# humanlongevity/tredparse

Measured on AMD Instinct MI355X. Metric: sample x TRED genotypes/sec at 30x 150bp, higher is better.
Workload: dtype int32 (SW) + f64 (likelihood)

## Files before the change

tredparse_amd/csrc/capi.hip:

```cpp
#include <algorithm>
#include <cstdarg>
#include <cstdio>
#include <cmath>
#include <cstdlib>
#include <cstring>
#include <ctime>
#include <string>
#include <vector>

#include <unistd.h>

#include "tredgpu_internal.h"
#include "inflater_internal.h"
#include "kmer_host.h"

using namespace tredgpu;

namespace {

struct Buf {
    void* p = nullptr;
    size_t cap = 0;
};

std::string g_create_error;

}

struct tredgpu_ctx {
    int device = 0;
    hipStream_t stream = nullptr;
    std::string err;
    std::vector<LadderDesc> h_ladders;
    Buf d_ladders, d_seq;
    int max_ladder_units = 0;
    Buf d_model;
    bool have_model = false;
    Buf ws_quads, ws_counter, ws_drop, ws_stats, ws_perm, ws_class, ws_ucnt, ws_bins, ws_best, ws_cnt;
    struct GridBufs { Buf pool, descs, items, counters, kde, unit_max; } grid;
    int* h_pin = nullptr;
    hipEvent_t sync_ev = nullptr;
    size_t grid_pool_bytes = GRID_POOL_BYTES;
    std::vector<Buf> st;
    struct PinBlock { uint8_t* p; size_t cap, used; };
    std::vector<PinBlock> pin;
    struct PinOut { void* host; const void* pinned; size_t bytes; };
    std::vector<PinOut> pin_out;
    struct Timer {
        std::vector<std::pair<hipEvent_t, hipEvent_t>> pool;
        size_t used = 0;
        int64_t launches = 0;
        double total_ms = 0;
    } timers[7];
};

namespace {

int fail(tredgpu_ctx* c, int code, const char* fmt, ...) {
    char buf[512];
    va_list ap;
    va_start(ap, fmt);
    vsnprintf(buf, sizeof buf, fmt, ap);
    va_end(ap);
    if (c) c->err = buf; else g_create_error = buf;
    return code;
}

int hip_rc(tredgpu_ctx* c, hipError_t e, const char* what) {
    return e == hipSuccess ? 0 : fail(c, -10, "%s: %s", what, hipGetErrorString(e));
}

#define HIPRC(c, expr) hip_rc((c), (expr), #expr)
#define HIPCHK(c, expr)                          \
    do {                                         \
        if (int rc_ = HIPRC(c, expr)) return rc_; \
    } while (0)

void timer_flush(tredgpu_ctx::Timer& t) {
    for (size_t i = 0; i < t.used; ++i) {
        float ms = 0;
        if (hipEventElapsedTime(&ms, t.pool[i].first, t.pool[i].second) == hipSuccess) {
            t.total_ms += ms;
            t.launches += 1;
        }
    }
    t.used = 0;
}

struct ScopedTimer {
    tredgpu_ctx* c;
    tredgpu_ctx::Timer& t;
    hipEvent_t stop = nullptr;
    ScopedTimer(tredgpu_ctx* c_, int which) : c(c_), t(c_->timers[which]) {
        if (t.used >= 256) {
            (void)hipStreamSynchronize(c->stream);
            timer_flush(t);
        }
        if (t.used == t.pool.size()) {
            hipEvent_t a = nullptr, b = nullptr;
            if (hipEventCreate(&a) != hipSuccess || hipEventCreate(&b) != hipSuccess) return;
            t.pool.emplace_back(a, b);
        }
        (void)hipEventRecord(t.pool[t.used].first, c->stream);
        stop = t.pool[t.used].second;
    }
    ~ScopedTimer() {
        if (stop) {
            (void)hipEventRecord(stop, c->stream);
            t.used += 1;
        }
    }
};

void* pin_alloc(tredgpu_ctx* c, size_t bytes) {
    bytes = (bytes + 63) & ~(size_t)63;
    for (auto& b : c->pin)
        if (b.cap - b.used >= bytes) { void* at = b.p + b.used; b.used += bytes; return at; }
    size_t cap = std::max<size_t>(bytes, (size_t)8 << 20);
    if (!c->pin.empty()) cap = std::max(cap, c->pin.back().cap * 2);
    uint8_t* p = nullptr;
    if (hipHostMalloc((void**)&p, cap, hipHostMallocDefault) != hipSuccess) return nullptr;
// ... 143 lines not shown
        const Staged& a = list[k];
        if (!a.dst || !a.bytes) continue;
        void* h;
        if ((rc = pin_for(c, a.bytes, &h))) break;
        rc = HIPRC(c, hipMemcpyAsync(h, c->st[k].p, a.bytes, hipMemcpyDeviceToHost, c->stream));
        if (!rc) c->pin_out.push_back({a.dst, h, a.bytes});
    }
    if (rc) {
        (void)stream_sync(c, false);
        return rc;
    }
    return HIPRC(c, stream_sync(c));
}

int check_unit(tredgpu_ctx* c, int g, const tredgpu_unit_params& u, const int32_t* unit_ladder, int32_t hist_stride,
               int64_t n_global_total, int64_t n_target_total, int32_t marg_stride, int limits[2]) {
    if (unit_ladder) {
        const int lad = unit_ladder[g];
        if (lad < 0 || lad >= (int)c->h_ladders.size()) return fail(c, -2, "unit %d: ladder %d not registered", g, lad);
        if (hist_stride <= c->h_ladders[lad].max_units)
            return fail(c, -2, "hist_stride %d must exceed the max_units %d of unit %d's ladder", hist_stride, c->h_ladders[lad].max_units, g);
    }
    limits[0] = std::max(limits[0], u.maxinsert);
    limits[1] = std::max(limits[1], u.n_target);
    if (u.n_global < 0 || u.n_target < 0 || u.pe_off < 0 || u.tl_off < 0 || (int64_t)u.pe_off + u.n_global > n_global_total ||
        (int64_t)u.tl_off + u.n_target > n_target_total)
        return fail(c, -2, "unit %d: paired-end slices out of range", g);
    if (marg_stride > 0 && marg_stride <= std::max(u.maxinsert, hist_stride)) return fail(c, -2, "marg_stride must exceed max(maxinsert, hist_stride)");
    return 0;
}

int host_max_len(tredgpu_ctx* c, const tredgpu_sw_params* p, const int32_t* read_len, int64_t n_reads, int* max_len) {
    int seen = 0;
    for (int64_t r = 0; r < n_reads; ++r) seen = std::max(seen, read_len[r]);
    if (seen > TREDGPU_MAX_READ_LEN) return fail(c, -5, "read of %d bp exceeds TREDGPU_MAX_READ_LEN=%d", seen, TREDGPU_MAX_READ_LEN);
    *max_len = std::max(p->max_read_len > 0 ? p->max_read_len : seen, 1);
    return check_sw_range(c, p, *max_len);
}

}

extern "C" {

#ifndef TREDGPU_SRC_HASH
#define TREDGPU_SRC_HASH "unknown"
#endif
const char* tredgpu_version(void) { return "tredgpu 0.6 (gfx950) src " TREDGPU_SRC_HASH; }

int tredgpu_create(int device_id, tredgpu_ctx** out) {
    if (!out) return fail(nullptr, -2, "out is NULL");
    *out = nullptr;
    int n = 0;
    hipError_t e = hipGetDeviceCount(&n);
    if (e != hipSuccess || n <= 0)
        return fail(nullptr, -3, "no HIP device available (%s); libtredgpu has no CPU fallback",
                    e == hipSuccess ? "device count 0" : hipGetErrorString(e));
    if (device_id < 0 || device_id >= n) return fail(nullptr, -2, "device %d out of range [0,%d)", device_id, n);
    tredgpu_ctx* c = new tredgpu_ctx();
    c->device = device_id;
    int lo_prio = 0, hi_prio = 0;
    const char* want = getenv("TREDGPU_CTX_PRIORITY");
    const bool high = want && strcmp(want, "high") == 0;
    const char* split = getenv("TREDGPU_CTX_CUS");
    if ((e = hipSetDevice(device_id)) != hipSuccess ||
        (e = (split && atoi(split) > 0) ? tredgpu_front::create_partitioned_stream(&c->stream, hipStreamDefault, 0, 1, device_id)
             : high && hipDeviceGetStreamPriorityRange(&lo_prio, &hi_prio) == hipSuccess
                 ? hipStreamCreateWithPriority(&c->stream, hipStreamDefault, hi_prio) : hipStreamCreate(&c->stream)) != hipSuccess) {
        delete c;
        return fail(nullptr, -10, "cannot initialise device %d: %s", device_id, hipGetErrorString(e));
    }
    if (const char* mb = getenv("TREDGPU_GRID_POOL_MB")) {
        const long v = atol(mb);
        if (v > 0) c->grid_pool_bytes = (size_t)v << 20;
    }
    *out = c;
    return 0;
}

void tredgpu_destroy(tredgpu_ctx* c) {
    if (!c) return;
    (void)hipSetDevice(c->device);
    (void)stream_sync(c);
    for (Buf* b : {&c->d_ladders, &c->d_seq, &c->d_model, &c->ws_quads, &c->ws_counter, &c->ws_drop,
                   &c->ws_stats, &c->ws_perm, &c->ws_class, &c->ws_ucnt, &c->ws_bins, &c->ws_best, &c->ws_cnt, &c->grid.pool, &c->grid.descs,
                   &c->grid.items, &c->grid.counters, &c->grid.kde, &c->grid.unit_max})
        release(*b);
    for (Buf& b : c->st) release(b);
    for (auto& t : c->timers)
        for (auto& ev : t.pool) { (void)hipEventDestroy(ev.first); (void)hipEventDestroy(ev.second); }
    if (c->h_pin) (void)hipHostFree(c->h_pin);
    if (c->sync_ev) (void)hipEventDestroy(c->sync_ev);
    for (auto& b : c->pin) (void)hipHostFree(b.p);
    c->pin.clear();
    (void)hipStreamDestroy(c->stream);
    delete c;
}

const char* tredgpu_last_error(const tredgpu_ctx* c) { return c ? c->err.c_str() : g_create_error.c_str(); }

int tredgpu_sync(tredgpu_ctx* c) {
    if (!c) return -2;
    HIPCHK(c, hipSetDevice(c->device));
    HIPCHK(c, stream_sync(c));
    return 0;
}

void* tredgpu_get_stream(tredgpu_ctx* c) { return c ? (void*)c->stream : nullptr; }

int tredgpu_reset_timing(tredgpu_ctx* c) {
    if (!c) return -2;
    HIPCHK(c, hipSetDevice(c->device));
    HIPCHK(c, stream_sync(c));
    for (auto& t : c->timers) { t.used = 0; t.launches = 0; t.total_ms = 0; }
    if (c->ws_stats.p) HIPCHK(c, hipMemsetAsync(c->ws_stats.p, 0, SW_STAT_SLOTS * 8 * sizeof(unsigned long long), c->stream));
    return 0;
}

int tredgpu_get_sw_counters(tredgpu_ctx* c, uint64_t out[8]) {
    if (!c || !out) return -2;
    HIPCHK(c, hipSetDevice(c->device));
    for (int i = 0; i < 8; ++i) out[i] = 0;
    if (c->ws_stats.p) {
        std::vector<uint64_t> slots((size_t)SW_STAT_SLOTS * 8);
        HIPCHK(c, hipMemcpyAsync(slots.data(), c->ws_stats.p, slots.size() * sizeof(uint64_t), hipMemcpyDeviceToHost, c->stream));
        HIPCHK(c, stream_sync(c));
        for (int k = 0; k < SW_STAT_SLOTS; ++k)
            for (int i = 0; i < 8; ++i) out[i] += slots[(size_t)k * 8 + i];
    }
    HIPCHK(c, stream_sync(c));
    return 0;
}

int tredgpu_get_timing(tredgpu_ctx* c, int which, int64_t* launches, double* total_ms) {
    if (!c) return -2;
    if (which < 0 || which > 6) return fail(c, -2, "which must be one of TREDGPU_KERNEL_*");
    HIPCHK(c, hipSetDevice(c->device));
    HIPCHK(c, stream_sync(c));
    timer_flush(c->timers[which]);
    if (launches) *launches = c->timers[which].launches;
    if (total_ms) *total_ms = c->timers[which].total_ms;
    return 0;
}

int tredgpu_set_ladders(tredgpu_ctx* c, int32_t n, const char* const* prefix, const char* const* repeat,
                        const char* const* suffix, const int32_t* max_units) {
    if (!c) return -2;
    if (n < 0 || (n > 0 && (!prefix || !repeat || !suffix || !max_units))) return fail(c, -2, "bad ladder arguments");
    HIPCHK(c, hipSetDevice(c->device));
    std::vector<uint32_t> seq;
    auto append = [&seq](const std::vector<int8_t>& v) {
        const int off = (int)seq.size();
        seq.resize(seq.size() + (v.size() + 7) / 8 + 1, 0x44444444u);
        for (size_t i = 0; i < v.size(); ++i) {
            uint32_t& w = seq[off + i / 8];
            w = (w & ~(0xFu << ((i % 8) * 4))) | ((uint32_t)v[i] << ((i % 8) * 4));
        }
        return off;
    };
    std::vector<LadderDesc> lad((size_t)n);
    int max_u = 0;
    for (int i = 0; i < n; ++i) {
        std::vector<int8_t> P, Rp, S;
        encode(prefix[i], P);
        encode(repeat[i], Rp);
        encode(suffix[i], S);
        const int mu = max_units[i];
        LadderDesc& d = lad[i];
// ... 61 lines not shown
    HIPCHK(c, hipSetDevice(c->device));
    std::vector<ModelConst> mbuf(1);
    ModelConst& m = mbuf[0];
    memcpy(m.step, step_pdf, sizeof m.step);
    memcpy(m.w, stutter_w, sizeof m.w);
    m.gc = gc;
    m.score = score;
    m.small = std::exp(-10.0);
    m.really_small = std::exp(-100.0);
    m.logsmall = std::log(m.small);
    for (int n = 0; n < GRID_LFACT; ++n) m.lfact[n] = std::lgamma((double)n + 1);
    int rc;
    if ((rc = ensure(c, c->d_model, sizeof m))) return rc;
    HIPCHK(c, stream_sync(c));
    HIPCHK(c, hipMemcpy(c->d_model.p, &m, sizeof m, hipMemcpyHostToDevice));
    c->have_model = true;
    return 0;
}

int64_t tredgpu_pack_reads(const char* seqs, const int64_t* seq_off, int64_t n_reads, uint32_t* packed_out,
                           int64_t* word_off_out, int32_t* len_out) {
    if (n_reads < 0 || (n_reads > 0 && (!seqs || !seq_off))) return -2;
    int64_t w = 0;
    for (int64_t r = 0; r < n_reads; ++r) {
        const int64_t L = seq_off[r + 1] - seq_off[r];
        if (L < 0 || L > 0x7fffffff) return -2;
        const int64_t nb = (L + 15) >> 4, nm = (L + 31) >> 5;
        if (word_off_out) word_off_out[r] = w;
        if (len_out) len_out[r] = (int32_t)L;
        if (packed_out) {
            uint32_t* rec = packed_out + w;
            for (int64_t k = 0; k < nb + nm; ++k) rec[k] = 0;
            const char* s = seqs + seq_off[r];
            for (int64_t i = 0; i < L; ++i) {
                const int code = base_code(s[i]);
                if (code == 4) rec[nb + (i >> 5)] |= 1u << (i & 31);
                else rec[i >> 4] |= (uint32_t)code << ((i & 15) * 2);
            }
        }
        w += nb + nm;
    }
    if (word_off_out) word_off_out[n_reads] = w;
    return w;
}


static int run_sw_device(tredgpu_ctx* c, const uint32_t* packed, const int64_t* read_off, const int32_t* read_len,
                         int64_t n_reads, const int32_t* unit_read_off, const int32_t* unit_ladder,
                         int32_t n_units, const tredgpu_sw_params* p, int max_len, uint8_t* out_tag,
                         int16_t* out_h, int16_t* out_score, int16_t* out_dump, int32_t dump_templates) {
    if (n_reads == 0 || n_units == 0) return 0;
    const int n_ladders = (int)c->h_ladders.size();
    const int64_t max_quads = sw_max_quads(n_reads, n_ladders);
    int rc;
    if ((rc = ensure(c, c->ws_quads, (size_t)max_quads * sizeof(Quad)))) return rc;
    if ((rc = ensure(c, c->ws_counter, 64))) return rc;
    SwArgs a;
    a.packed = packed;
    a.read_off = read_off;
    a.read_len = read_len;
    a.unit_read_off = unit_read_off;
    a.unit_ladder = unit_ladder;
    a.ladders = (const LadderDesc*)c->d_ladders.p;
    a.seqw = (const uint32_t*)c->d_seq.p;
    a.quads = (const Quad*)c->ws_quads.p;
    a.n_quads = (const int32_t*)c->ws_counter.p;
    a.out_tag = out_tag;
    a.out_h = out_h;
    a.out_score = out_score;
    a.out_dump = out_dump;
    a.dump_templates = dump_templates;
    a.n_units = n_units;
    a.n_ladders = n_ladders;
    a.max_rows = 16 * rows_for(max_len);
    a.p = *p;
    a.stats = nullptr;
    if ((rc = ensure(c, c->ws_perm, (size_t)n_reads * sizeof(int32_t)))) return rc;
    if ((rc = ensure(c, c->ws_class, (size_t)n_reads))) return rc;
    a.perm = (const int32_t*)c->ws_perm.p;
    if ((rc = ensure(c, c->ws_ucnt, sw_unit_cnt_bytes(n_units)))) return rc;
    if ((rc = ensure(c, c->ws_bins, sw_bin_bytes(n_ladders)))) return rc;
    if ((rc = ensure(c, c->ws_best, (size_t)n_reads * sizeof(int32_t)))) return rc;
    if ((rc = ensure(c, c->ws_cnt, (size_t)n_reads * sizeof(int32_t)))) return rc;
    a.best = (int32_t*)c->ws_best.p;
    a.read_cnt = (const int32_t*)c->ws_cnt.p;
    if (c->ws_stats.p == nullptr) {
        if ((rc = ensure(c, c->ws_stats, SW_STAT_SLOTS * 8 * sizeof(unsigned long long)))) return rc;
        HIPCHK(c, hipMemsetAsync(c->ws_stats.p, 0, SW_STAT_SLOTS * 8 * sizeof(unsigned long long), c->stream));
    }
    a.stats = (unsigned long long*)c->ws_stats.p;
    const int rows = rows_for(max_len);
    auto build_quads = [&](int pass) {
        return launch_build_quads(a, pass, rows, (uint8_t*)c->ws_class.p, (int32_t*)c->ws_cnt.p, (int32_t*)c->ws_perm.p,
                                  (Quad*)c->ws_quads.p, (int32_t*)c->ws_counter.p, (int32_t*)c->ws_ucnt.p,
                                  (int32_t*)c->ws_bins.p, n_ladders, max_quads, c->stream);
    };
    HIPCHK(c, build_quads(0));
    {
        ScopedTimer tm(c, TREDGPU_KERNEL_SW);
        bool generic = false;
        bool two_strands = false;
        for (const LadderDesc& d : c->h_ladders) {
            for (int s2 = 0; s2 < d.n_strands; ++s2) generic = generic || (d.max_units > 0 && d.blen[s2] * p->match >= 30);
            two_strands = two_strands || d.n_strands >= 2;
        }
        HIPCHK(c, launch_sw_ladder(a, rows, generic, max_quads, c->stream));
        if (out_dump == nullptr && two_strands) {
            HIPCHK(c, build_quads(1));
            HIPCHK(c, launch_sw_ladder(a, rows, generic, max_quads, c->stream));
        }
    }
    return 0;
}

int tredgpu_sw_classify(tredgpu_ctx* c, int mem, const uint32_t* packed, const int64_t* read_off,
                        const int32_t* read_len, int64_t n_reads, const int32_t* unit_read_off,
                        const int32_t* unit_ladder, int32_t n_units, const tredgpu_sw_params* params,
                        uint8_t* out_tag, int16_t* out_h, int16_t* out_score, int16_t* out_dump,
                        int32_t dump_templates) {
    if (!c) return -2;
    int rc;
    if ((rc = check_sw_params(c, params))) return rc;
    if (n_reads < 0 || n_units < 0) return fail(c, -2, "negative sizes");
    if (n_reads > 0 && (!packed || !read_off || !read_len || !unit_read_off || !unit_ladder || !out_tag || !out_h || !out_score))
        return fail(c, -2, "NULL array argument");
    if (c->h_ladders.empty()) return fail(c, -4, "no ladders registered (tredgpu_set_ladders)");
    if (out_dump && dump_templates <= 0) return fail(c, -2, "dump_templates must be > 0 with out_dump");
    HIPCHK(c, hipSetDevice(c->device));
    int max_len = params->max_read_len;
    if (mem == TREDGPU_MEM_DEVICE) {
        if (max_len <= 0) max_len = TREDGPU_ASSUMED_READ_LEN;
        if (out_dump) HIPCHK(c, hipMemsetAsync(out_dump, 0xFF, (size_t)n_reads * dump_templates * 6 * sizeof(int16_t), c->stream));
        return run_sw_device(c, packed, read_off, read_len, n_reads, unit_read_off, unit_ladder, n_units, params,
                             max_len, out_tag, out_h, out_score, out_dump, dump_templates);
    }
    if (mem != TREDGPU_MEM_HOST) return fail(c, -2, "mem must be TREDGPU_MEM_HOST or TREDGPU_MEM_DEVICE");
    if (n_reads == 0) return 0;
    if (unit_read_off[0] != 0 || unit_read_off[n_units] != n_reads) return fail(c, -2, "unit_read_off must span [0,n_reads]");
    for (int g = 0; g < n_units; ++g) {
        if (unit_read_off[g + 1] < unit_read_off[g]) return fail(c, -2, "unit_read_off not monotone at %d", g);
        if (unit_ladder[g] < 0 || unit_ladder[g] >= (int)c->h_ladders.size()) return fail(c, -2, "unit %d: ladder %d not registered", g, unit_ladder[g]);
    }
    if ((rc = host_max_len(c, params, read_len, n_reads, &max_len))) return rc;
    const uint32_t* d_packed; const int64_t* d_off; const int32_t* d_len; const int32_t* d_uoff; const int32_t* d_ulad;
    uint8_t* d_tag; int16_t* d_h; int16_t* d_score; int16_t* d_dump = nullptr;
    const size_t n = (size_t)n_reads, g = (size_t)n_units, dump_n = out_dump ? n * dump_templates * 6 : 0;
    const std::vector<Staged> list = {
        arr_in(d_packed, packed, (size_t)read_off[n_reads]), arr_in(d_off, read_off, n + 1), arr_in(d_len, read_len, n),
        arr_in(d_uoff, unit_read_off, g + 1), arr_in(d_ulad, unit_ladder, g),
        arr_out(d_tag, out_tag, n), arr_out(d_h, out_h, n), arr_out(d_score, out_score, n),
        out_dump ? arr_out(d_dump, out_dump, dump_n) : absent,
    };
    rc = stage(c, list);
    if (!rc && out_dump) rc = HIPRC(c, hipMemsetAsync(d_dump, 0xFF, dump_n * sizeof(int16_t), c->stream));
    if (!rc) rc = run_sw_device(c, d_packed, d_off, d_len, n_reads, d_uoff, d_ulad, n_units, params, max_len, d_tag, d_h,
                                d_score, d_dump, dump_templates);
    return finish(c, list, rc);
}

int tredgpu_tally(tredgpu_ctx* c, int mem, const uint8_t* tag, const int16_t* h, int64_t n_reads,
                  const int32_t* unit_read_off, int32_t n_units, const int32_t* read_pair_id, int32_t hist_stride,
                  int32_t* full_cnt, int32_t* pref_cnt, int32_t* rept_cnt) {
    if (!c) return -2;
    if (n_reads < 0 || n_units < 0 || hist_stride <= 0) return fail(c, -2, "bad sizes");
    if (n_units > 0 && (!unit_read_off || !full_cnt || !pref_cnt || !rept_cnt)) return fail(c, -2, "NULL array argument");
    if (n_reads > 0 && (!tag || !h)) return fail(c, -2, "NULL array argument");
    HIPCHK(c, hipSetDevice(c->device));
    int rc;
// ... 369 lines not shown
```

tredparse_amd/csrc/kmer_host.h:

```cpp
#pragma once
#include <cstdint>
#include <vector>

namespace kmer_host {

constexpr int BITS_WORDS = 128;
constexpr int CLS_WORDS = 512;

template <class Vec>
inline bool holds_n(const Vec& v) {
    for (size_t i = 0; i < v.size(); ++i)
        if (v[i] > 3) return true;
    return false;
}

template <class Vec>
inline bool build_tables(const Vec& head, const Vec& repeat, const Vec& branch, int max_units, std::vector<uint32_t>& bits,
                         std::vector<uint32_t>& cls) {
    bits.assign(BITS_WORDS, 0u);
    cls.clear();
    const bool with_n = max_units > 0 && (holds_n(head) || holds_n(repeat) || holds_n(branch));
    std::vector<uint8_t> fewest(4096, 15);
    std::vector<bool> seen((size_t)1 << 18, false);
    Vec t;
    for (int u = 1; u <= max_units; ++u) {
        t.assign(head.begin(), head.end());
        for (int k = 0; k < u; ++k) t.insert(t.end(), repeat.begin(), repeat.end());
        t.insert(t.end(), branch.begin(), branch.end());
        for (size_t i = 0; i + 6 <= t.size(); ++i) {
            uint32_t code = 0, mask = 0;
            int wild[6], nw = 0;
            for (int k = 0; k < 6; ++k) {
                if (t[i + k] > 3) { wild[nw++] = k; mask |= 1u << k; }
                else code |= (uint32_t)(t[i + k] & 3) << (2 * k);
            }
            const uint32_t key = code | mask << 12;
            if (seen[key]) continue;
            seen[key] = true;
            for (uint32_t f = 0; f < (1u << (2 * nw)); ++f) {
                uint32_t cf = code;
                for (int j = 0; j < nw; ++j) cf |= ((f >> (2 * j)) & 3u) << (2 * wild[j]);
                bits[cf >> 5] |= 1u << (cf & 31);
                if (nw < fewest[cf]) fewest[cf] = (uint8_t)nw;
            }
        }
    }
    if (with_n) {
        cls.assign(CLS_WORDS, 0u);
        for (uint32_t w = 0; w < 4096; ++w)
            if (fewest[w] != 15) cls[w >> 3] |= (uint32_t)fewest[w] << (4 * (w & 7));
    }
    return with_n;
}

}
```

tredparse_amd/csrc/sw_ladder.hip:

```cpp
#include "tredgpu_internal.h"

namespace tredgpu {
namespace {

constexpr int KSH = 18;
constexpr int KONE = 1 << KSH;
constexpr int PAYMASK = KONE - 1;
constexpr int NEG = -(1 << 30);
constexpr int PADNEG = -64 * KONE;
constexpr int CNT_UNFILTERED = 0x7FFF;
#ifndef SW_EXIT_BOUND
#define SW_EXIT_BOUND 1
#endif

__device__ __forceinline__ int kmer_weight(int cnt, int jsum) { return cnt - (jsum + 5) / 6; }
__device__ __forceinline__ int kmer_cap(int w, int match) { return (w + 5) * match; }

template <int CTRL>
__device__ __forceinline__ int dpp_row_shr(int old, int x) {
    return __builtin_amdgcn_update_dpp(old, x, CTRL, 0xF, 0xF, false);
}

__device__ __forceinline__ int add3_vsv(int v0, int s1, int v2) {
    int d;
    asm("v_add3_u32 %0, %1, %2, %3" : "=v"(d) : "v"(v0), "s"(s1), "v"(v2));
    return d;
}
__device__ __forceinline__ int add_sv(int s0, int v1) {
    int d;
    asm("v_add_u32 %0, %1, %2" : "=v"(d) : "s"(s0), "v"(v1));
    return d;
}
__device__ __forceinline__ int max3(int a, int b, int c) { return max(max(a, b), c); }

__device__ __forceinline__ int row_scan_max(int x) {
    x = max(x, dpp_row_shr<0x111>(x, x));
    x = max(x, dpp_row_shr<0x112>(x, x));
    x = max(x, dpp_row_shr<0x114>(x, x));
    x = max(x, dpp_row_shr<0x118>(x, x));
    return x;
}

template <int CTRL>
__device__ __forceinline__ void pair_step(int& k, int& s) {
    const int tk = dpp_row_shr<CTRL>(k, k);
    const int ts = dpp_row_shr<CTRL>(s, s);
    const bool c = tk > k;
    k = c ? tk : k;
    s = c ? ts : s;
}

template <int R>
struct Rows {
    int S[4][R];
    int rowc0;
};

struct Track {
    int bestkey;
    int beststart;
    int ceil;
};

__device__ __forceinline__ int row_excl_scan_max(int x) {
    constexpr int IMIN = -2147483647 - 1;
    x = max(x, dpp_row_shr<0x111>(IMIN, x));
    x = max(x, dpp_row_shr<0x112>(IMIN, x));
    x = max(x, dpp_row_shr<0x114>(IMIN, x));
    x = max(x, dpp_row_shr<0x118>(IMIN, x));
    return dpp_row_shr<0x111>(NEG, x);
}

__device__ __forceinline__ int row_max_all(int x) {
    constexpr int IMIN = -2147483647 - 1;
    x = max(x, __builtin_amdgcn_update_dpp(IMIN, x, 0x121, 0xF, 0xF, false));
    x = max(x, __builtin_amdgcn_update_dpp(IMIN, x, 0x122, 0xF, 0xF, false));
    x = max(x, __builtin_amdgcn_update_dpp(IMIN, x, 0x124, 0xF, 0xF, false));
    x = max(x, __builtin_amdgcn_update_dpp(IMIN, x, 0x128, 0xF, 0xF, false));
    return x;
}

__device__ __forceinline__ int row_scan_max_fused(int x) {
    constexpr int IMIN = -2147483647 - 1;
    x = max(x, dpp_row_shr<0x111>(IMIN, x));
    x = max(x, dpp_row_shr<0x112>(IMIN, x));
    x = max(x, dpp_row_shr<0x114>(IMIN, x));
    x = max(x, dpp_row_shr<0x118>(IMIN, x));
    return x;
}

__device__ __forceinline__ int row_excl_scan_max_e10(int x, int* E, const int* q, int before) {
    int fin;
    asm("v_max_i32 %2, %2, %12\n\t"
        "v_max_i32 %3, %3, %13\n\t"
        "v_max_i32_dpp %0, %0, %0 row_shr:1 row_mask:0xf bank_mask:0xf\n\t"
// ... 437 lines not shown
                    const int bestS = best >> 12, bestU = 511 - ((best >> 3) & 511);
                    const int need_score = max(max(min(L, Tlen) >> 1, 30), u >= bestU ? bestS + 1 : bestS);
                    if (__builtin_amdgcn_ballot_w64(valid && jl == 15 && (ks >> KSH) >= need_score) == 0) {
                        cnt_ends += 1u << 8;
                        ++u;
                        if (__builtin_amdgcn_ballot_w64(valid && jl == 15 && still_open(u)) == 0) return true;
                        return false;
                    }
                }
                resolve_best<R>(T, row0, row0g, geK, rowbuf);
                bk = T.bestkey, bs = T.beststart;
                const bool c = m > bk;
                ++cnt_ends;
                bk = c ? m : bk;
                bs = c ? st : bs;
                {
                    const int bkm = row_max_all(bk);
                    bs = row_max_all(bk == bkm ? bs : -1);
                    bk = bkm;
                }
                if (with_sfx) {
                    const int sk = wb[(2 * R) * PS], ss = wb[(2 * R + 1) * PS];
                    const int k3 = sk - ((col + 1) << 9), s3 = ss + ((col + 1) << 9);
                    const bool c3 = sk != floor_key && (k3 > bk || (k3 == bk && s3 > bs));
                    bk = c3 ? k3 : bk;
                    bs = c3 ? s3 : bs;
                }
            } else {
                cnt_ends += 1u << 16;
                resolve_best<R>(T, row0, row0g, geK, rowbuf);
                bk = T.bestkey, bs = T.beststart;
                pair_step<0x111>(bk, bs);
                pair_step<0x112>(bk, bs);
                pair_step<0x114>(bk, bs);
                pair_step<0x118>(bk, bs);
            }
            const int score = bk >> KSH;
            const int ref_end = 511 - ((bk >> 9) & 511), read_end = 511 - (bk & 511);
            const int ref_begin = (bs >> 9) & 511, read_begin = bs & 511;
            const int min_len = min(L, Tlen) >> 1;
            const int min_score = max(min_len, 30);
            const bool pass = score >= min_score && (read_end - read_begin + 1) >= min_len;
            const int aL = ref_begin, aR = Tlen - ref_end - 1, bL = read_begin, bR = L - read_end - 1;
            const int hang = min(min(aR + bL, aL + bR), min(aL + aR, bL + bR));
            const bool prefix_read = ref_begin < flank;
            const bool suffix_read = ref_end > Tlen - flank - 1;
            int tag;
            if (hang >= flank) tag = TREDGPU_TAG_HANG;
            else if (prefix_read) tag = suffix_read ? TREDGPU_TAG_FULL : TREDGPU_TAG_PREF;
            else if (suffix_read) tag = TREDGPU_TAG_POST;
            else if (u >= mu_rept - 1 && u * period <= L) tag = TREDGPU_TAG_REPT;
            else tag = TREDGPU_TAG_NONE;
            if (!pass) tag = TREDGPU_TAG_NONE;
            const int cand = (score << 9 | (511 - u)) << 3;
            best = tag != TREDGPU_TAG_NONE && cand > (best | 7) ? cand | tag : best;
            if (full_dump && valid && jl == 15) {
                const int k = max_units > 0 ? 2 * (u - 1) + s : 0;
                if (k < a.dump_templates) {
                    int16_t* d = a.out_dump + ((int64_t)a.perm[q_first + job] * a.dump_templates + k) * 6;
                    const bool hit = score > 0 && bk != floor_key;
                    d[0] = (int16_t)(hit ? score : 0);
                    d[1] = (int16_t)(hit ? ref_begin : -1);
                    d[2] = (int16_t)(hit ? ref_end : -1);
                    d[3] = (int16_t)(hit ? read_begin : 0);
                    d[4] = (int16_t)(hit ? read_end : 0);
                    d[5] = (int16_t)tag;
                }
            }
            ++u;
            if (!full_dump && __builtin_amdgcn_ballot_w64(valid && jl == 15 && still_open(u)) == 0) return true;
            return false;
        };
        int ok_run = 0;
        auto steady_exit = [&](const uint32_t ends_before) -> bool {
            if (full_dump || ((cnt_ends ^ ends_before) & 0xFF00u) == 0) { ok_run = 0; return false; }
#if SW_EXIT_BOUND
            if constexpr (!GENERIC && (R == 7 || R == 10)) if (__builtin_amdgcn_ballot_w64(best >= 0) != 0) {
                const int c = next_end - period;
                const int r0 = (lane_now() & 15) * R;
                const int bestS = best >> 12, bestU = 511 - ((best >> 3) & 511);
                const int need = max(max(min(L, alen + period * u + blen) >> 1, 30), u >= bestU ? bestS + 1 : bestS);
                int nt = (L - 1 - r0) * mK - need * KONE - (r0 + c) * geK;
                uint32_t lo = 0x3FFFFu;
#pragma unroll
                for (int r = 0; r < R; ++r) {
                    lo = min(lo, min((uint32_t)(H[r] + nt) & 0x8003FE00u, (uint32_t)(E[r] + nt - geK) & 0x8003FE00u));
                    nt -= mK + geK;
                    asm volatile("" : "+v"(nt), "+v"(lo));
                }
                if (__builtin_amdgcn_ballot_w64(lo < ((uint32_t)(alen + period) << 9)) == 0) return true;
            }
#endif
            const uint32_t thr = (uint32_t)(alen + (ok_run ? period : 0)) << 9;
            uint32_t lo = 0x3FFFFu;
#pragma unroll
            for (int r = 0; r < R; ++r) lo = min(lo, min((uint32_t)H[r] & 0x3FE00u, (uint32_t)E[r] & 0x3FE00u));
            if (__builtin_amdgcn_ballot_w64(lo < thr) != 0) { ok_run = 0; return false; }
            if (ok_run) return true;
            ok_run = 1;
            return false;
        };
        if (period == 3 && max_units > 0) {
            int col = 0;
            for (; col < alen; ++col) {
                sweep_letter<R>(letter_from(tw, col), J, H, E, T, col, row0, geK, c0, row0g, rowbuf);
                ++cnt_cols;
            }
            int P0[R], P1[R], P2[R];
            pick_profile<R>(J, letter_from(tw, alen), geK, P0);
            pick_profile<R>(J, letter_from(tw, alen + 1), geK, P1);
            pick_profile<R>(J, letter_from(tw, alen + 2), geK, P2);
            for (;;) {
                sweep_at<R>(J, P0, H, E, T, col, row0, geK, c0, row0g, rowbuf);
                sweep_at<R>(J, P1, H, E, T, col + 1, row0, geK, c0, row0g, rowbuf);
                sweep_at<R>(J, P2, H, E, T, col + 2, row0, geK, c0, row0g, rowbuf);
                col += 3;
                cnt_cols += 3;
                const uint32_t ends_before = cnt_ends;
                if (template_end(col - 1) || col >= ncols || steady_exit(ends_before)) break;
            }
        } else {
            for (int col = 0; col < ncols; ++col) {
                sweep_letter<R>(letter_from(tw, col), J, H, E, T, col, row0, geK, c0, row0g, rowbuf);
                ++cnt_cols;
                if (col != next_end) continue;
                const uint32_t ends_before = cnt_ends;
                if (template_end(col) || (max_units > 0 && steady_exit(ends_before))) break;
            }
        }
    }
    const int lane_e = lane_now();
    if (a.stats != nullptr && lane_e < 7) {
        const int n_trunk_cols = (int)(cnt_cols & 0xFFFFu), n_cont_cols = (int)(cnt_cols >> 16);
        const int vals[7] = {n_trunk_cols, n_cont_cols, (int)(cnt_ends & 0xFFu), (int)((cnt_ends >> 8) & 0xFFu),
                             (int)(cnt_ends >> 16), 1, (n_trunk_cols + n_cont_cols) * q_count};
        int v = 0;
#pragma unroll
        for (int k = 0; k < 7; ++k) v = lane_e == k ? vals[k] : v;
        atomicAdd(a.stats + (size_t)(blockIdx.x & (SW_STAT_SLOTS - 1)) * 8 + lane_e, (unsigned long long)v);
    }
    if ((lane_e >> 4) < q_count && (lane_e & 15) == 15) {
        const int64_t rd = (int64_t)a.perm[q_first + (lane_e >> 4)];
        int bestTag = best < 0 ? TREDGPU_TAG_NONE : best & 7;
        int bestU = 511 - ((best >> 3) & 511), bestS = best >> 12;
        if (too_long) bestTag = TREDGPU_TAG_INVALID, bestU = 0, bestS = 0;
        a.out_tag[rd] = (uint8_t)bestTag;
        a.out_h[rd] = (int16_t)(bestTag == TREDGPU_TAG_NONE ? 0 : bestU);
        a.out_score[rd] = (int16_t)(bestTag == TREDGPU_TAG_NONE ? 0 : bestS);
        a.best[rd] = best;
    }
}

constexpr int BIN_STRIDE = 16;
constexpr int SW_LEVELS = 32;
constexpr int UNIT_BINS = SW_LEVELS;
constexpr int KEY_NONE = 0xFF;
__device__ __forceinline__ int level_key(int cnt) { return SW_LEVELS - 1 - min(SW_LEVELS - 1, cnt / 6); }
__device__ __forceinline__ int kmer_threshold(const tredgpu_sw_params& p) {
    return min(p.mismatch, p.gap_open) >= 5 * p.match ? (30 + p.match - 1) / p.match - 5 : 0;
}

__device__ __forceinline__ void claim_bin_runs(const int* hist, int lad, int g, int32_t* unit_cnt, int32_t* bin_total) {
    for (int k = threadIdx.x; k < UNIT_BINS; k += (int)blockDim.x) {
        const int n = hist[k];
        int at = 0;
        if (n) at = atomicAdd(bin_total + ((size_t)lad * UNIT_BINS + k) * BIN_STRIDE, n);
        unit_cnt[(size_t)g * UNIT_BINS + k] = at;
    }
}

template <bool NCLS>
__device__ __forceinline__ void kmer_counts(const uint32_t* rec, int L, const uint32_t* bm, const uint32_t* kc, int& cnt0, int& cnt1) {
    const int nb = (L + 15) >> 4;
    uint32_t prev = 0, mprev = 0;
    cnt0 = cnt1 = 0;
    int j0 = 0, j1 = 0;
    for (int wi = 0; wi < nb; ++wi) {
        const uint32_t w = rec[wi];
        const uint32_t m = (rec[nb + (wi >> 1)] >> ((wi & 1) * 16)) & 0xffffu;
        uint32_t b0 = 0, b1 = 0;
        const uint32_t mm = m << 5 | mprev >> 11;
        const uint32_t hn = mm | mm >> 1 | mm >> 2 | mm >> 3 | mm >> 4 | mm >> 5;
        const int left = L - wi * 16;
        uint32_t cm = left >= 16 ? 0xffffu : (1u << left) - 1u;
        if (wi == 0) cm &= ~0x1fu;
        const uint32_t plain = cm & ~hn;
#pragma unroll
        for (int j = 0; j < 16; ++j) {
            const uint32_t t = j > 5 ? w >> (2 * (j - 5)) : (j == 5 ? w : __builtin_amdgcn_alignbit(w, prev, 32 - 2 * (5 - j)));
            const uint32_t at = __builtin_amdgcn_ubfe(t, 5, 7);
            b0 = (__builtin_amdgcn_ubfe(bm[at], t, 1) << j) | b0;
            b1 = (__builtin_amdgcn_ubfe(bm[128 + at], t, 1) << j) | b1;
            if (NCLS) {
                const uint32_t at4 = __builtin_amdgcn_ubfe(t, 3, 9), sh = (t & 7u) << 2;
                const bool use = (plain >> j) & 1u;
                j0 += use ? (int)__builtin_amdgcn_ubfe(kc[at4], sh, 4) : 0;
                j1 += use ? (int)__builtin_amdgcn_ubfe(kc[512 + at4], sh, 4) : 0;
            }
        }
        cnt0 += __builtin_popcount((b0 | hn) & cm);
        cnt1 += __builtin_popcount((b1 | hn) & cm);
        prev = w;
        mprev = m;
    }
    if (NCLS) {
        cnt0 = kmer_weight(cnt0, j0);
        cnt1 = kmer_weight(cnt1, j1);
    }
}

__global__ __launch_bounds__(64) void read_class_kernel(SwArgs a, uint8_t* read_key, int32_t* read_cnt, int32_t* unit_cnt,
                                                          int32_t* bin_total) {
    const int g = blockIdx.x;
    if (g >= a.n_units) return;
    const int lad = min(max(a.unit_ladder[g], 0), a.n_ladders - 1);
    const LadderDesc* ld = a.ladders + lad;
    const bool full_dump = a.out_dump != nullptr;
    const int thr = kmer_threshold(a.p);
    const bool filt = !full_dump && thr > 0 && ld->kmer_ok != 0 && ld->max_units > 0;
    const int r0 = a.unit_read_off[g], r1 = a.unit_read_off[g + 1];
    __shared__ uint32_t bm[2][128];
    __shared__ uint32_t kc[2][512];
    __shared__ int hist[UNIT_BINS];
    const bool ncls = filt && ld->kmer_n != 0;
    if (filt) {
        for (int k = threadIdx.x; k < 256; k += (int)blockDim.x) bm[k >> 7][k & 127] = a.seqw[ld->kmer_off[k >> 7] + (k & 127)];
    }
    if (ncls) {
        for (int k = threadIdx.x; k < 1024; k += (int)blockDim.x) kc[k >> 9][k & 511] = a.seqw[ld->kcls_off[k >> 9] + (k & 511)];
    }
    for (int k = threadIdx.x; k < UNIT_BINS; k += (int)blockDim.x) hist[k] = 0;
    __syncthreads();
    for (int rd = r0 + (int)threadIdx.x; rd < r1; rd += (int)blockDim.x) {
        int cnt0 = CNT_UNFILTERED, cnt1 = CNT_UNFILTERED;
        const int L = a.read_len[rd];
        if (filt && L <= a.max_rows) {
            if (ncls) kmer_counts<true>(a.packed + a.read_off[rd], L, &bm[0][0], &kc[0][0], cnt0, cnt1);
            else kmer_counts<false>(a.packed + a.read_off[rd], L, &bm[0][0], nullptr, cnt0, cnt1);
        }
        read_cnt[rd] = cnt0 | cnt1 << 16;
        a.best[rd] = -1;
        if (cnt0 >= thr) {
            const int key = level_key(cnt0);
            read_key[rd] = (uint8_t)key;
            atomicAdd(&hist[key], 1);
        } else {
            read_key[rd] = (uint8_t)KEY_NONE;
            a.out_tag[rd] = TREDGPU_TAG_NONE;
            a.out_h[rd] = 0;
            a.out_score[rd] = 0;
        }
    }
    __syncthreads();
    claim_bin_runs(hist, lad, g, unit_cnt, bin_total);
}

__global__ __launch_bounds__(64) void repack_kernel(SwArgs a, uint8_t* read_key, const int32_t* read_cnt, int32_t* unit_cnt,
                                                      int32_t* bin_total, int kcap_in_kernel) {
    const int g = blockIdx.x;
    if (g >= a.n_units) return;
    const int lad = min(max(a.unit_ladder[g], 0), a.n_ladders - 1);
    const LadderDesc* ld = a.ladders + lad;
    const int thr = kmer_threshold(a.p);
    const bool with_kcap = kcap_in_kernel && thr > 0 && ld->kmer_ok != 0;
    const bool two_strands = ld->n_strands >= 2;
    const int first_T = ld->alen[1] + ld->period * (ld->max_units > 0 ? 1 : 0) + ld->blen[1];
    const int r0 = a.unit_read_off[g], r1 = a.unit_read_off[g + 1];
    __shared__ int hist[UNIT_BINS];
    __shared__ int n_pass;
    for (int k = threadIdx.x; k < UNIT_BINS; k += (int)blockDim.x) hist[k] = 0;
    if (threadIdx.x == 0) n_pass = 0;
    __syncthreads();
    for (int rd = r0 + (int)threadIdx.x; rd < r1; rd += (int)blockDim.x) {
        const int L = a.read_len[rd];
        const int cnt1 = (int)((uint32_t)read_cnt[rd] >> 16);
        const bool counted = cnt1 != CNT_UNFILTERED;
        const int kcap = with_kcap && counted ? kmer_cap(cnt1, a.p.match) : 1 << 20;
        const int cap = min(kcap, L * a.p.match);
        const int min_score = max(min(L, first_T) >> 1, 30);
        const bool open = max(min_score, (a.best[rd] >> 12) + 1) <= cap;
        const bool go = two_strands && L <= a.max_rows && cnt1 >= thr && open;
        int key = KEY_NONE;
        if (go) {
            key = level_key(cnt1);
            atomicAdd(&hist[key], 1);
            atomicAdd(&n_pass, 1);
        }
        read_key[rd] = (uint8_t)key;
    }
    __syncthreads();
    claim_bin_runs(hist, lad, g, unit_cnt, bin_total);
    if (threadIdx.x == 0 && a.stats != nullptr && n_pass)
        atomicAdd(a.stats + (size_t)(g & (SW_STAT_SLOTS - 1)) * 8 + 7, (unsigned long long)n_pass);
}

__global__ __launch_bounds__(1024) void bin_scan_kernel(int32_t* bins, int n_bins, int32_t* n_quads) {
    __shared__ int cs[1024], cq[1024];
    const int t = threadIdx.x;
    const int chunk = (n_bins + 1023) / 1024;
    const int b0 = min(t * chunk, n_bins), b1 = min(b0 + chunk, n_bins);
    int slots = 0, quads = 0;
    for (int b = b0; b < b1; ++b) {
        const int n = bins[(size_t)b * BIN_STRIDE];
        slots += n;
        quads += (n + 3) >> 2;
    }
    cs[t] = slots; cq[t] = quads;
    __syncthreads();
    if (t == 0) {
        int s = 0, q = 0;
        for (int k = 0; k < 1024; ++k) { const int a_ = cs[k], b_ = cq[k]; cs[k] = s; cq[k] = q; s += a_; q += b_; }
        bins[(size_t)n_bins * BIN_STRIDE + 2] = q;
        *n_quads = q;
    }
    __syncthreads();
    int slot = cs[t], quad = cq[t];
    for (int b = b0; b < b1; ++b) {
        int32_t* e = bins + (size_t)b * BIN_STRIDE;
        e[1] = slot;
        e[2] = quad;
        slot += e[0];
// ... 171 lines not shown
```

tredparse_amd/csrc/tredgpu_internal.h:

```cpp
#pragma once
#include <hip/hip_runtime.h>
#include <stdint.h>
#include "../../include/tredgpu.h"
#include "grid_host.h"

namespace tredgpu {

struct LadderDesc {
    int32_t alen[2];
    int32_t blen[2];
    int32_t trunk_off[2];
    int32_t branch_off[2];
    int32_t period;
    int32_t max_units;
    int32_t n_strands;
    int32_t kmer_ok;
    int32_t kmer_off[2];
    int32_t kmer_n;
    int32_t kcls_off[2];
};

struct Quad {
    int32_t ladder;
    int32_t first;
    int32_t count;
    int32_t strands;
};

struct SwArgs {
    const uint32_t* packed;
    const int64_t* read_off;
    const int32_t* read_len;
    const int32_t* unit_read_off;
    const int32_t* unit_ladder;
    const LadderDesc* ladders;
    const uint32_t* seqw;
    const Quad* quads;
    const int32_t* perm;
    const int32_t* n_quads;
    uint8_t* out_tag;
    int16_t* out_h;
    int16_t* out_score;
    int16_t* out_dump;
    int32_t dump_templates;
    int32_t n_units;
    int32_t n_ladders;
    int32_t max_rows;
    tredgpu_sw_params p;
    unsigned long long* stats;
    int32_t* best;
    const int32_t* read_cnt;
};

constexpr int SW_STAT_SLOTS = 1024;

hipError_t launch_build_quads(const SwArgs& a, int pass, int rows_per_lane, uint8_t* read_key, int32_t* read_cnt, int32_t* perm,
                              Quad* quads, int32_t* n_quads, int32_t* unit_cnt, int32_t* bins, int n_ladders, int64_t max_quads,
                              hipStream_t s);
size_t sw_bin_bytes(int n_ladders);
size_t sw_unit_cnt_bytes(int n_units);
int64_t sw_max_quads(int64_t n_reads, int n_ladders);
hipError_t launch_sw_ladder(const SwArgs& a, int rows_per_lane, bool generic, int64_t max_quads, hipStream_t s);
hipError_t launch_tally(const uint8_t* tag, const int16_t* h, int64_t n_reads,
                        const int32_t* unit_read_off, int32_t n_units, const int32_t* read_pair_id,
                        int32_t hist_stride, int32_t* full_cnt, int32_t* pref_cnt,
                        int32_t* rept_cnt, uint8_t* scratch_drop, hipStream_t s);

struct ModelConst {
    double step[6][37];
    double w[5];
    double gc, score;
    double small;
    double really_small;
    double logsmall;
    double lfact[4096];
};
constexpr int GRID_LFACT = 4096;

struct GridArgs {
    const tredgpu_unit_params* units;
    int32_t n_units;
    int32_t hist_stride;
    const int32_t* full_cnt;
    const int32_t* pref_cnt;
    const int32_t* rept_cnt;
    const int32_t* global_lens;
    const int32_t* target_lens;
    tredgpu_call* calls;
    const int64_t* grid_off;
    double* grid_dump;
    double* marg;
    int32_t marg_stride;
    const ModelConst* model;
    const int64_t* joint_off;
    double* joint;
    int32_t* joint_n;
    double* joint_total;
    double* kde_pdf;
    int32_t* kde_status;
    double* unit_pdf;
    int32_t* unit_kde_rc;
    int32_t max_target;
};
constexpr size_t GRID_POOL_BYTES = (size_t)12 << 30;
constexpr int GRID_UNIT_DEFERRED = 100;

hipError_t launch_pe_kde(const GridArgs& a, hipStream_t s);
hipError_t launch_unit_max(const tredgpu_unit_params* units, int n_units, int* out, hipStream_t s);

struct GridDescs;
struct GridItems;
struct GridCounterBlock;
struct GridWorkspace {
    GridPlan plan;
    GridDescs* descs;
    double* pool;
    GridItems* items;
    GridCounterBlock* counters;
    double* kde_pdf;
    int32_t* kde_rc;
};
const int32_t* grid_deferred(const GridWorkspace& w);
enum class GridPhase { KDE = TREDGPU_KERNEL_GRID_KDE, PREPARE = TREDGPU_KERNEL_GRID_PREPARE, PAIRS = TREDGPU_KERNEL_GRID_PAIRS,
                       REDUCE = TREDGPU_KERNEL_GRID_REDUCE };
hipError_t launch_grid_phase(const GridArgs& a, const GridWorkspace& w, int pass, GridPhase phase, hipStream_t s);

}
```

Baseline: 1.685 million.

## Tighten SW early-exit bound using per-lane k-mer tail counts

During k-mer counting, each read now gets per-lane counts of the remaining k-mer hits in its tail. They are stored in a new workspace buffer and computed with shared-memory scratch. The Smith-Waterman early-exit check uses these counts to bound each lane's best possible remaining score more tightly, so hopeless ladder units can be abandoned sooner. The exit path also returns immediately instead of falling through to the later check. The price is extra work and memory traffic in the counting pass and a per-read global load in the exit check.

After: 1.746 million (median of 6 runs). 1.04x the previous value.

```diff
diff --git a/tredparse_amd/csrc/capi.hip b/tredparse_amd/csrc/capi.hip
--- a/tredparse_amd/csrc/capi.hip
+++ b/tredparse_amd/csrc/capi.hip
@@ -36,7 +36,7 @@
     int max_ladder_units = 0;
     Buf d_model;
     bool have_model = false;
-    Buf ws_quads, ws_counter, ws_drop, ws_stats, ws_perm, ws_class, ws_ucnt, ws_bins, ws_best, ws_cnt;
+    Buf ws_quads, ws_counter, ws_drop, ws_stats, ws_perm, ws_class, ws_ucnt, ws_bins, ws_best, ws_cnt, ws_tail;
     struct GridBufs { Buf pool, descs, items, counters, kde, unit_max; } grid;
     int* h_pin = nullptr;
     hipEvent_t sync_ev = nullptr;
@@ -346,7 +346,7 @@
     (void)hipSetDevice(c->device);
     (void)stream_sync(c);
     for (Buf* b : {&c->d_ladders, &c->d_seq, &c->d_model, &c->ws_quads, &c->ws_counter, &c->ws_drop,
-                   &c->ws_stats, &c->ws_perm, &c->ws_class, &c->ws_ucnt, &c->ws_bins, &c->ws_best, &c->ws_cnt, &c->grid.pool, &c->grid.descs,
+                   &c->ws_stats, &c->ws_perm, &c->ws_class, &c->ws_ucnt, &c->ws_bins, &c->ws_best, &c->ws_cnt, &c->ws_tail, &c->grid.pool, &c->grid.descs,
                    &c->grid.items, &c->grid.counters, &c->grid.kde, &c->grid.unit_max})
         release(*b);
     for (Buf& b : c->st) release(b);
@@ -574,8 +574,10 @@
     if ((rc = ensure(c, c->ws_bins, sw_bin_bytes(n_ladders)))) return rc;
     if ((rc = ensure(c, c->ws_best, (size_t)n_reads * sizeof(int32_t)))) return rc;
     if ((rc = ensure(c, c->ws_cnt, (size_t)n_reads * sizeof(int32_t)))) return rc;
+    if ((rc = ensure(c, c->ws_tail, (size_t)n_reads * 2 * kmer_host::TAIL_LANES))) return rc;
     a.best = (int32_t*)c->ws_best.p;
     a.read_cnt = (const int32_t*)c->ws_cnt.p;
+    a.read_tail = (uint8_t*)c->ws_tail.p;
     if (c->ws_stats.p == nullptr) {
         if ((rc = ensure(c, c->ws_stats, SW_STAT_SLOTS * 8 * sizeof(unsigned long long)))) return rc;
         HIPCHK(c, hipMemsetAsync(c->ws_stats.p, 0, SW_STAT_SLOTS * 8 * sizeof(unsigned long long), c->stream));
diff --git a/tredparse_amd/csrc/kmer_host.h b/tredparse_amd/csrc/kmer_host.h
--- a/tredparse_amd/csrc/kmer_host.h
+++ b/tredparse_amd/csrc/kmer_host.h
@@ -53,4 +53,32 @@
     return with_n;
 }
 
+#if defined(__HIPCC__)
+#define KMER_HD __host__ __device__
+#else
+#define KMER_HD
+#endif
+constexpr int TAIL_LANES = 16;
+constexpr int TAIL_SAT = 254;
+constexpr int TAIL_NONE = 255;
+
+KMER_HD inline uint32_t tail_entry(uint32_t end_mask, int before) { return (end_mask & 0xffffu) | (uint32_t)before << 16; }
+
+KMER_HD inline int tail_count(const uint32_t* entries, int stride, int nb, int total, int R, int lane) {
+    const int e = lane * R + 5;
+    const int w = e >> 4;
+    if (w >= nb) return 0;
+    const uint32_t en = entries[w * stride];
+    const int t = total - (int)(en >> 16) - __builtin_popcount(en & ((1u << (e & 15)) - 1u));
+    return t > TAIL_SAT ? TAIL_SAT : t;
 }
+
+KMER_HD inline void tail_pack(const uint32_t* entries, int stride, int nb, int total, int R, uint32_t out[4]) {
+    for (int k = 0; k < 4; ++k) {
+        uint32_t v = 0;
+        for (int b = 0; b < 4; ++b) v |= (uint32_t)tail_count(entries, stride, nb, total, R, 4 * k + b) << (8 * b);
+        out[k] = v;
+    }
+}
+
+}
diff --git a/tredparse_amd/csrc/sw_ladder.hip b/tredparse_amd/csrc/sw_ladder.hip
--- a/tredparse_amd/csrc/sw_ladder.hip
+++ b/tredparse_amd/csrc/sw_ladder.hip
@@ -1,4 +1,5 @@
 #include "tredgpu_internal.h"
+#include "kmer_host.h"
 
 namespace tredgpu {
 namespace {
@@ -10,7 +11,10 @@
 constexpr int PADNEG = -64 * KONE;
 constexpr int CNT_UNFILTERED = 0x7FFF;
 #ifndef SW_EXIT_BOUND
-#define SW_EXIT_BOUND 1
+#define SW_EXIT_BOUND 2
+#endif
+#ifndef SW_EXIT_FALLTHROUGH
+#define SW_EXIT_FALLTHROUGH 0
 #endif
 
 __device__ __forceinline__ int kmer_weight(int cnt, int jsum) { return cnt - (jsum + 5) / 6; }
@@ -614,13 +618,31 @@
                 const int need = max(max(min(L, alen + period * u + blen) >> 1, 30), u >= bestU ? bestS + 1 : bestS);
                 int nt = (L - 1 - r0) * mK - need * KONE - (r0 + c) * geK;
                 uint32_t lo = 0x3FFFFu;
+#if SW_EXIT_BOUND >= 2
+                const int lnx = lane_now();
+                const int wt = (lnx >> 4) < q_count ? (int)a.read_tail[((int64_t)a.perm[q_first + (lnx >> 4)] * 2 + s) * kmer_host::TAIL_LANES + (lnx & 15)]
+                                                    : kmer_host::TAIL_NONE;
+                int nt2 = min(5 + wt, L) * mK - need * KONE - (r0 + c) * geK;
+#pragma unroll
+                for (int r = 0; r < R; ++r) {
+                    const int t = min(nt, nt2);
+                    lo = min(lo, min((uint32_t)(H[r] + t) & 0x8003FE00u, (uint32_t)(E[r] + t - geK) & 0x8003FE00u));
+                    nt -= mK + geK;
+                    nt2 -= geK;
+                    asm volatile("" : "+v"(nt), "+v"(nt2), "+v"(lo));
+                }
+#else
 #pragma unroll
                 for (int r = 0; r < R; ++r) {
                     lo = min(lo, min((uint32_t)(H[r] + nt) & 0x8003FE00u, (uint32_t)(E[r] + nt - geK) & 0x8003FE00u));
                     nt -= mK + geK;
                     asm volatile("" : "+v"(nt), "+v"(lo));
                 }
+#endif
                 if (__builtin_amdgcn_ballot_w64(lo < ((uint32_t)(alen + period) << 9)) == 0) return true;
+#if !SW_EXIT_FALLTHROUGH
+                return false;
+#endif
             }
 #endif
             const uint32_t thr = (uint32_t)(alen + (ok_run ? period : 0)) << 9;
@@ -701,8 +723,10 @@
     }
 }
 
-template <bool NCLS>
-__device__ __forceinline__ void kmer_counts(const uint32_t* rec, int L, const uint32_t* bm, const uint32_t* kc, int& cnt0, int& cnt1) {
+constexpr int TAIL_WORDS = 10;
+template <bool NCLS, bool TAIL>
+__device__ __forceinline__ void kmer_counts(const uint32_t* rec, int L, const uint32_t* bm, const uint32_t* kc, int& cnt0, int& cnt1,
+                                            uint32_t* tl = nullptr, int R = 0, uint8_t* tail = nullptr) {
     const int nb = (L + 15) >> 4;
     uint32_t prev = 0, mprev = 0;
     cnt0 = cnt1 = 0;
@@ -730,10 +754,21 @@
                 j1 += use ? (int)__builtin_amdgcn_ubfe(kc[512 + at4], sh, 4) : 0;
             }
         }
+        if (TAIL) {
+            tl[wi * 64] = kmer_host::tail_entry((b0 | hn) & cm, cnt0);
+            tl[(TAIL_WORDS + wi) * 64] = kmer_host::tail_entry((b1 | hn) & cm, cnt1);
+        }
         cnt0 += __builtin_popcount((b0 | hn) & cm);
         cnt1 += __builtin_popcount((b1 | hn) & cm);
         prev = w;
         mprev = m;
+    }
+    if (TAIL) {
+        uint32_t t0[4], t1[4];
+        kmer_host::tail_pack(tl, 64, nb, cnt0, R, t0);
+        kmer_host::tail_pack(tl + TAIL_WORDS * 64, 64, nb, cnt1, R, t1);
+        reinterpret_cast<uint4*>(tail)[0] = make_uint4(t0[0], t0[1], t0[2], t0[3]);
+        reinterpret_cast<uint4*>(tail)[1] = make_uint4(t1[0], t1[1], t1[2], t1[3]);
     }
     if (NCLS) {
         cnt0 = kmer_weight(cnt0, j0);
@@ -755,6 +790,9 @@
     __shared__ uint32_t kc[2][512];
     __shared__ int hist[UNIT_BINS];
     const bool ncls = filt && ld->kmer_n != 0;
+    __shared__ uint32_t tl[2 * TAIL_WORDS * 64];
+    const int tail_R = a.max_rows / 16;
+    const bool tails = filt && (tail_R == 7 || tail_R == 10);
     if (filt) {
         for (int k = threadIdx.x; k < 256; k += (int)blockDim.x) bm[k >> 7][k & 127] = a.seqw[ld->kmer_off[k >> 7] + (k & 127)];
     }
@@ -766,9 +804,19 @@
     for (int rd = r0 + (int)threadIdx.x; rd < r1; rd += (int)blockDim.x) {
         int cnt0 = CNT_UNFILTERED, cnt1 = CNT_UNFILTERED;
         const int L = a.read_len[rd];
+        uint8_t* const tail = a.read_tail + (int64_t)rd * (2 * kmer_host::TAIL_LANES);
         if (filt && L <= a.max_rows) {
-            if (ncls) kmer_counts<true>(a.packed + a.read_off[rd], L, &bm[0][0], &kc[0][0], cnt0, cnt1);
-            else kmer_counts<false>(a.packed + a.read_off[rd], L, &bm[0][0], nullptr, cnt0, cnt1);
+            if (tails) {
+                if (ncls) kmer_counts<true, true>(a.packed + a.read_off[rd], L, &bm[0][0], &kc[0][0], cnt0, cnt1, tl + threadIdx.x, tail_R, tail);
+                else kmer_counts<false, true>(a.packed + a.read_off[rd], L, &bm[0][0], nullptr, cnt0, cnt1, tl + threadIdx.x, tail_R, tail);
+            } else {
+                if (ncls) kmer_counts<true, false>(a.packed + a.read_off[rd], L, &bm[0][0], &kc[0][0], cnt0, cnt1);
+                else kmer_counts<false, false>(a.packed + a.read_off[rd], L, &bm[0][0], nullptr, cnt0, cnt1);
+            }
+        }
+        if (!(tails && L <= a.max_rows)) {
+            reinterpret_cast<uint4*>(tail)[0] = make_uint4(~0u, ~0u, ~0u, ~0u);
+            reinterpret_cast<uint4*>(tail)[1] = make_uint4(~0u, ~0u, ~0u, ~0u);
         }
         read_cnt[rd] = cnt0 | cnt1 << 16;
         a.best[rd] = -1;
diff --git a/tredparse_amd/csrc/tredgpu_internal.h b/tredparse_amd/csrc/tredgpu_internal.h
--- a/tredparse_amd/csrc/tredgpu_internal.h
+++ b/tredparse_amd/csrc/tredgpu_internal.h
@@ -50,6 +50,7 @@
     unsigned long long* stats;
     int32_t* best;
     const int32_t* read_cnt;
+    uint8_t* read_tail;
 };
 
 constexpr int SW_STAT_SLOTS = 1024;
```
